# miguelmartin75/txt2vid

Measured on AMD Instinct MI355X. Metric: TGANv2 GAN train throughput (G+D steps x global batch), 16x64x64 videos/sec, higher is better.
Workload: dtype f32; 1 GPU; BASELINE configs[1]: unconditional TGANv2 16x64x64x1, per-GPU batch 32, fp32, RSGAN + GP 0.5, Adam 2e-4 (0.5,0.999), 1 D + 1 G step, subsample_input pyramid 8/16/32/64; global_batch=32, per_gpu_batch=32, parallelism=dp1

## Files before the change

### include/t2v_hip.h

```cpp
#ifndef T2V_HIP_H
#define T2V_HIP_H

#include <stddef.h>
#include <stdint.h>

#ifdef __cplusplus
extern "C" {
#endif

#define T2V_OK 0
#define T2V_EINVAL (-1)
#define T2V_ELAUNCH (-2)

#define T2V_MAX_TAPS 27

typedef struct {
    int32_t N, Cin, D, H, W, Cout;
    int32_t ntaps;
    int8_t dz[T2V_MAX_TAPS], dy[T2V_MAX_TAPS], dx[T2V_MAX_TAPS];
    int8_t pad_[3];
} t2v_conv_geom;

#define T2V_MAX_GROUPS 8
typedef struct {
// ... 28 lines not shown
    int32_t block_begin;
    int32_t bx, by;
    int8_t taps[T2V_MAX_TAPS];
    int8_t pad_[5];
} t2v_pack_job;
int t2v_pack_job_bytes(void);
int t2v_pack_job_groups(int T, int ntaps, int mode);
int t2v_pack_multi(const void* table , int njobs, int total_blocks, void* stream);

int t2v_conv_fwd(const float* x, const float* wp, const float* bias, float* y, float* ws, const t2v_conv_geom* g,
                 int flags, void* stream);
int64_t t2v_conv_fwd_ws_floats(const t2v_conv_geom* g);

int64_t t2v_conv_wgrad_slab_floats(const t2v_conv_geom* g, int T);
int t2v_conv_wgrad(const float* x, const float* gy, float* dw, float* slab, const t2v_conv_geom* g,
                   const int32_t* taps, int T, int flags, void* stream);

int64_t t2v_conv_fwd_grouped_ws_floats(const t2v_conv_group* groups, int ngroups, int Cin, int Cout);
int t2v_conv_fwd_grouped(const t2v_conv_group* groups, int ngroups, int Cin, int Cout, const float* wp,
                         const float* bias, float* ws, int flags, void* stream);
int64_t t2v_conv_wgrad_grouped_slab_floats(const t2v_conv_group* groups, int ngroups, int Cin, int Cout, int kD,
                                           int kH, int kW);
int t2v_conv_wgrad_grouped(const t2v_conv_group* groups, int ngroups, int Cin, int Cout, int kD, int kH, int kW,
                           float* dw, float* slab, int flags, void* stream);
#define T2V_WGRAD_MAX_SRC 6
typedef struct {
    const float* slab;
    const float* bias_slab;
    int32_t ntaps, S;
    int8_t map[T2V_MAX_TAPS];
    int8_t pad_[5];
    int64_t tap_stride;
    int64_t split_stride;
} t2v_wgrad_src;
typedef struct {
    float* dw;
    float* dbias;
    int64_t CoCi;
    int32_t T, Cout, nsrc;
    int32_t accum, accum_bias;
    int32_t kind;
    int32_t block_begin, nblocks;
    int32_t tap_major;
    int32_t pad_;
    t2v_wgrad_src src[T2V_WGRAD_MAX_SRC];
} t2v_wgrad_dest;
int t2v_conv_wgrad_grouped_partial(const t2v_conv_group* groups, int ngroups, int Cin, int Cout, int kD, int kH, int kW,
                                   float* slab, int want_bias, int flags, t2v_wgrad_src* out_src, void* stream);
int t2v_wgrad_dest_bytes(void);
int t2v_wgrad_reduce_multi(const void* table , int ndest, int total_blocks, void* stream);

int t2v_conv_fwd_plan(const t2v_conv_group* groups, int ngroups, int Cin, int Cout, int flags, int32_t* out);
int t2v_conv_wgrad_plan(const t2v_conv_group* groups, int ngroups, int Cin, int Cout, int kD, int kH, int kW, int32_t* out);
int64_t t2v_conv_wgrad_grouped_bias_slab_floats(const t2v_conv_group* groups, int ngroups, int Cin, int Cout, int kD,
                                                int kH, int kW);
int t2v_conv_wgrad_grouped_bias(const t2v_conv_group* groups, int ngroups, int Cin, int Cout, int kD, int kH, int kW,
                                float* dw, float* dbias, float* slab, int flags, void* stream);

int t2v_pack_weight_bf16(const float* w, void* wpb, int Cout, int Cin, int T, const int32_t* taps, int ntaps, int mode, void* stream);
int t2v_conv_fwd_grouped_bf16_ok(const t2v_conv_group* groups, int ngroups, int Cin, int Cout);
int t2v_conv_fwd_bf16_plan(const t2v_conv_group* groups, int ngroups, int Cin, int Cout, int flags, int32_t* out);
int t2v_conv_fwd_grouped_bf16(const t2v_conv_group* groups, int ngroups, int Cin, int Cout, const void* wpb, const float* bias,
                              float* ws, int flags, void* stream);

int64_t t2v_channel_sum_ws_floats(int N, int C, int64_t S);
int t2v_channel_sum(const float* x, float* out, float* ws, int N, int C, int64_t S, int accum, void* stream);
int64_t t2v_channel_sum_grouped_ws_floats(const t2v_conv_group* groups, int ngroups, int C);
int t2v_channel_sum_grouped(const t2v_conv_group* groups, int ngroups, int C, float* out, float* ws, int accum, void* stream);

int t2v_relu(const float* x, float* y, int64_t n, void* stream);
int t2v_relu_mask(const float* g, const float* x, float* gx, int64_t n, void* stream);
int t2v_add(const float* a, const float* b, float* y, int64_t n, void* stream);
int t2v_axpby(float alpha, const float* a, float beta, const float* b, float* y, int64_t n, void* stream);
int t2v_fill(float* y, float v, int64_t n, void* stream);
int t2v_tanh(const float* x, float* y, int64_t n, void* stream);
int t2v_tanh_bwd(const float* g, const float* y, float* gx, int64_t n, void* stream);

int t2v_avgpool3d(const float* x, const float* x2, float* y, int NC, int D, int H, int W, int Do, int Ho, int Wo,
                  const int32_t k[3], const int32_t s[3], const int32_t p[3], void* stream);
int t2v_avgpool3d_bwd(const float* gy, float* gx, int NC, int D, int H, int W, int Do, int Ho, int Wo,
                      const int32_t k[3], const int32_t s[3], const int32_t p[3], void* stream);
typedef struct t2v_pool_job {
    const float* x; const float* x2; float* y;
    const float* add;
    int32_t NC, D, H, W, Do, Ho, Wo;
    int32_t k[3], s[3], p[3];
} t2v_pool_job;
int t2v_avgpool3d_multi(const t2v_pool_job* jobs, int njobs, void* stream);
int t2v_avgpool3d_bwd_multi(const t2v_pool_job* jobs, int njobs, void* stream);

int t2v_rowsum(const float* x, float* y, int64_t rows, int64_t S, void* stream);
int t2v_rowbcast(const float* g, float* gx, int64_t rows, int64_t S, void* stream);

int t2v_upsample2x(const float* x, float* y, int64_t planes, int H, int W, void* stream);
int t2v_upsample2x_bwd(const float* gy, float* gx, int64_t planes, int H, int W, void* stream);
int t2v_upsample2x_add(const float* x, const float* h, float* y, int64_t planes, int H, int W, void* stream);

int64_t t2v_bn_ws_floats(int N, int C, int64_t S);
int t2v_bn_plan(int N, int C, int64_t S, int32_t* out );
int t2v_bn_stats(const float* x, float* stats, float* running_mean, float* running_var, float* ws, int N, int C,
                 int64_t S, float momentum, float eps, void* stream);
int t2v_bn_apply(const float* x, const float* stats, const float* gamma, const float* beta, float* y,
                 int N, int C, int64_t S, int relu, void* stream);
int t2v_bn_bwd(const float* gy, const float* x, const float* y, const float* stats, const float* gamma,
               float* gx, float* ggamma, float* gbeta, float* ws , int N, int C, int64_t S,
               int relu, void* stream);
// ... 278 lines not shown
```

### txt2vid_amd/_lib.py

```python
import ctypes as C
import os

_HERE = os.path.dirname(os.path.abspath(__file__))
LIB_PATH = os.environ.get('T2V_LIB') or os.path.join(_HERE, 'csrc', 'libt2v_hip.so')

MAX_TAPS = 27


class ConvGeom(C.Structure):
    _fields_ = [('N', C.c_int32), ('Cin', C.c_int32), ('D', C.c_int32), ('H', C.c_int32), ('W', C.c_int32),
                ('Cout', C.c_int32), ('ntaps', C.c_int32),
                ('dz', C.c_int8 * MAX_TAPS), ('dy', C.c_int8 * MAX_TAPS), ('dx', C.c_int8 * MAX_TAPS),
                ('pad_', C.c_int8 * 3)]


class ConvGroup(C.Structure):
    _fields_ = [('x', C.c_void_p), ('y', C.c_void_p), ('mask', C.c_void_p), ('N', C.c_int32), ('D', C.c_int32), ('H', C.c_int32), ('W', C.c_int32),
                ('ntaps', C.c_int32), ('dstride', C.c_int32), ('ydstride', C.c_int32), ('yoff', C.c_int32), ('Dy', C.c_int32),
                ('dz', C.c_int8 * MAX_TAPS), ('dy', C.c_int8 * MAX_TAPS), ('dx', C.c_int8 * MAX_TAPS), ('widx', C.c_int8 * MAX_TAPS)]


class AdamJob(C.Structure):
    _fields_ = [('p', C.c_void_p), ('g', C.c_void_p), ('m', C.c_void_p), ('v', C.c_void_p), ('n', C.c_int64)]

# ... 50 lines not shown

class AugMember(C.Structure):
    _fields_ = [('x', C.c_void_p), ('y', C.c_void_p), ('u', C.c_void_p), ('N', C.c_int32), ('C', C.c_int32), ('T', C.c_int32),
                ('S', C.c_int32), ('row_stride', C.c_int32), ('rows', C.c_int32), ('policy', C.c_int32), ('reserved', C.c_int32)]


class AdaLevel(C.Structure):
    _fields_ = [('real', C.c_void_p), ('fake', C.c_void_p), ('count', C.c_int32), ('reserved', C.c_int32)]


class LecamGrad(C.Structure):
    _fields_ = [('real', C.c_void_p), ('fake', C.c_void_p), ('d_real', C.c_void_p), ('d_fake', C.c_void_p), ('count', C.c_int32),
                ('reserved', C.c_int32)]


class ProjMember(C.Structure):
    _fields_ = [('g', C.c_void_p), ('f', C.c_void_p), ('s', C.c_void_p), ('base', C.c_void_p), ('out', C.c_void_p), ('b', C.c_int32),
                ('reserved', C.c_int32)]


class MbstdMember(C.Structure):
    _fields_ = [('f', C.c_void_p), ('g', C.c_void_p * 2), ('base', C.c_void_p * 2), ('gam', C.c_void_p), ('y', C.c_void_p * 2),
                ('stat', C.c_void_p), ('out', C.c_void_p), ('b', C.c_int32), ('seg', C.c_int32)]


MAX_GROUPS = 8
_P = C.c_void_p
_I = C.c_int
_L = C.c_int64
_F = C.c_float
_I3 = C.POINTER(C.c_int32)
_G = C.POINTER(ConvGeom)

SIGNATURES = {
    't2v_pack_weight': [_P, _P, _I, _I, _I, _I3, _I, _I, _P],
    't2v_pack_job_bytes': [],
    't2v_pack_multi': [_P, _I, _I, _P],
    't2v_pack_job_groups': [_I, _I, _I],
    't2v_pack_weight_into': [_P, _P, _I, _I, _I, _I3, _I, _I, _I, _I, _I, _I, _P],
    't2v_conv_fwd': [_P, _P, _P, _P, _P, _G, _I, _P],
    't2v_conv_fwd_ws_floats': [_G],
    't2v_conv_wgrad_slab_floats': [_G, _I],
    't2v_conv_fwd_grouped_ws_floats': [_P, _I, _I, _I],
    't2v_conv_fwd_grouped': [_P, _I, _I, _I, _P, _P, _P, _I, _P],
    't2v_conv_wgrad_grouped_slab_floats': [_P, _I, _I, _I, _I, _I, _I],
    't2v_conv_fwd_plan': [_P, _I, _I, _I, _I, _I3],
    't2v_nonlocal_ok': [_I, _I],
    't2v_nonlocal_fwd': [_P, _P, _P, _P, _P, _I, _I, _I, _I, _I, _P],
    't2v_nonlocal_bwd': [_P, _P, _P, _P, _P, _P, _P, _P, _P, _P, _I, _I, _I, _I, _I, _P],
    't2v_conv_wgrad_grouped_partial': [_P, _I, _I, _I, _I, _I, _I, _P, _I, _I, _P, _P],
    't2v_wgrad_dest_bytes': [],
    't2v_wgrad_reduce_multi': [_P, _I, _I, _P],
    't2v_conv_wgrad_plan': [_P, _I, _I, _I, _I, _I, _I, _I3],
    't2v_pack_weight_bf16': [_P, _P, _I, _I, _I, _P, _I, _I, _P],
    't2v_conv_fwd_grouped_bf16_ok': [_P, _I, _I, _I],
    't2v_conv_fwd_bf16_plan': [_P, _I, _I, _I, _I, _I3],
    't2v_conv_fwd_grouped_bf16': [_P, _I, _I, _I, _P, _P, _P, _I, _P],
    't2v_conv_wgrad_grouped': [_P, _I, _I, _I, _I, _I, _I, _P, _P, _I, _P],
    't2v_conv_wgrad_grouped_bias_slab_floats': [_P, _I, _I, _I, _I, _I, _I],
    't2v_conv_wgrad_grouped_bias': [_P, _I, _I, _I, _I, _I, _I, _P, _P, _P, _I, _P],
    't2v_conv_wgrad': [_P, _P, _P, _P, _G, _I3, _I, _I, _P],
    't2v_channel_sum_ws_floats': [_I, _I, _L],
    't2v_channel_sum': [_P, _P, _P, _I, _I, _L, _I, _P],
    't2v_channel_sum_grouped_ws_floats': [_P, _I, _I],
    't2v_channel_sum_grouped': [_P, _I, _I, _P, _P, _I, _P],
    't2v_relu': [_P, _P, _L, _P],
    't2v_relu_mask': [_P, _P, _P, _L, _P],
    't2v_add': [_P, _P, _P, _L, _P],
    't2v_axpby': [_F, _P, _F, _P, _P, _L, _P],
    't2v_fill': [_P, _F, _L, _P],
    't2v_tanh': [_P, _P, _L, _P],
    't2v_tanh_bwd': [_P, _P, _P, _L, _P],
    't2v_avgpool3d': [_P, _P, _P, _I, _I, _I, _I, _I, _I, _I, _I3, _I3, _I3, _P],
    't2v_avgpool3d_bwd': [_P, _P, _I, _I, _I, _I, _I, _I, _I, _I3, _I3, _I3, _P],
    't2v_avgpool3d_multi': [_P, _I, _P],
    't2v_avgpool3d_bwd_multi': [_P, _I, _P],
    't2v_rowsum': [_P, _P, _L, _L, _P],
    't2v_rowbcast': [_P, _P, _L, _L, _P],
    't2v_upsample2x': [_P, _P, _L, _I, _I, _P],
    't2v_upsample2x_bwd': [_P, _P, _L, _I, _I, _P],
    't2v_upsample2x_add': [_P, _P, _P, _L, _I, _I, _P],
    't2v_rsgan_mean_multi': [_P, _I, _P, _P],
    't2v_rsgan_mean_multi_bwd': [_P, _I, _P, _P],
    't2v_bn_ws_floats': [_I, _I, _L],
    't2v_bn_plan': [_I, _I, _L, _I3],
    't2v_bn_stats': [_P, _P, _P, _P, _P, _I, _I, _L, _F, _F, _P],
    't2v_bn_apply': [_P, _P, _P, _P, _P, _I, _I, _L, _I, _P],
    't2v_bn_bwd': [_P, _P, _P, _P, _P, _P, _P, _P, _P, _I, _I, _L, _I, _P],
    't2v_bn_train_fwd': [_P, _P, _P, _P, _P, _P, _P, _P, _I, _I, _L, _F, _F, _I, _P, _P],
    't2v_bn_train_bwd': [_P, _P, _P, _P, _P, _P, _P, _P, _P, _I, _I, _L, _I, _P],
    't2v_bn_train_fwd_up': [_P, _P, _P, _P, _P, _P, _P, _P, _I, _I, _I, _I, _F, _F, _I, _P, _P],
    't2v_bn_train_bwd_up': [_P, _P, _P, _P, _P, _P, _P, _P, _P, _I, _I, _I, _I, _I, _P],
    't2v_bn_train_bwd_add': [_P, _P, _P, _P, _P, _P, _P, _P, _P, _P, _I, _I, _I, _I, _I, _I, _P],
    't2v_bn_eval': [_P, _P, _P, _P, _P, _P, _I, _I, _L, _F, _I, _P],
    't2v_cbn_ws_floats': [_I, _I, _L],
    't2v_cbn_train_fwd': [_P] * 9 + [_I] * 9 + [_F, _F, _I, _P, _P],
    't2v_cbn_train_fwd_up': [_P] * 9 + [_I] * 9 + [_F, _F, _I, _P, _P],
    't2v_cbn_train_bwd': [_P] * 11 + [_I] * 9 + [_I, _P],
    't2v_cbn_train_bwd_up': [_P] * 11 + [_I] * 9 + [_I, _P],
    't2v_cbn_train_bwd_add': [_P] * 12 + [_I] * 9 + [_I, _I, _P],
    't2v_cbn_eval': [_P] * 7 + [_I] * 9 + [_F, _I, _P],
    't2v_lstm_gates': [_P, _P, _P, _P, _P, _I, _L, _P],
    't2v_lstm_gates_bwd': [_P, _P, _P, _P, _P, _P, _P, _I, _L, _P],
    't2v_skinny_gemm_splits': [_I, _I, _I],
    't2v_skinny_gemm_slab': [_P, _P, _P, _I, _I, _I, _P],
    't2v_lstm_gates_slab': [_P, _I, _P, _P, _P, _P, _P, _I, _I, _P],
# ... 125 lines not shown
```

### txt2vid_amd/csrc/conv.hip

```cpp
#include <hip/hip_runtime.h>
#include <stdint.h>
#include "../../include/t2v_hip.h"

typedef float f32x16 __attribute__((ext_vector_type(16)));

#ifdef T2V_STAMPS
__device__ unsigned long long* g_stamps = nullptr;
__device__ unsigned int g_stamps_cap = 0;
extern "C" int t2v_stamps_set(void* buf, unsigned int cap_records) {
    if (hipMemcpyToSymbol(HIP_SYMBOL(g_stamps), &buf, sizeof(buf)) != hipSuccess) return -1;
    if (hipMemcpyToSymbol(HIP_SYMBOL(g_stamps_cap), &cap_records, sizeof(cap_records)) != hipSuccess) return -1;
    return 0;
}
__device__ __forceinline__ unsigned long long stamp_now() {
    unsigned long long t;
    __builtin_amdgcn_sched_barrier(0);
    asm volatile("s_memtime %0\n\ts_waitcnt lgkmcnt(0)" : "=s"(t) :: "memory");
    __builtin_amdgcn_sched_barrier(0);
    return t;
}
#define STAMP(v) const unsigned long long v = stamp_now()
#define STAMP_ACC(acc, a, b) acc += (b) - (a)
#else
#define STAMP(v)
// ... 2369 lines not shown
        }
        if (mv) {
            py[(size_t)co * DHW] = a0;
            py[(size_t)(co + 1) * DHW] = a1;
            py[(size_t)(co + 2) * DHW] = a2;
            py[(size_t)(co + 3) * DHW] = a3;
        }
    }
}
static bool stem_ok(const t2v_conv_group* groups, int ngroups, int Cin, int Cout, int flags) {
    if ((Cin != 1 && Cin != 3) || Cout < 8 || Cout > 256 || (Cout % 4) != 0) return false;
    if (flags & (T2V_CONV_ACCUM | T2V_CONV_MASK_OUT)) return false;
    long M = 0;
    int taps = 0;
    for (int i = 0; i < ngroups; ++i) {
        if (groups[i].dstride == 2 || groups[i].ydstride == 2) return false;
        M += (long)groups[i].N * groups[i].D * groups[i].H * groups[i].W;
        if (groups[i].ntaps > taps) taps = groups[i].ntaps;
    }
    return M >= 65536 && taps > 18;
}

static bool thin_two_pass(const t2v_conv_group* groups, int ngroups, int Cin, int Cout, int nslots) {
    if (Cout != 1 || nslots < 9 || Cin < 16 || nslots * Cin > THIN_MAX_W) return false;
    long M = 0;
    for (int i = 0; i < ngroups; ++i) M += (long)groups[i].N * groups[i].D * groups[i].H * groups[i].W;
    return M >= 16384;
}

static bool thin_ok(const t2v_conv_group* groups, int ngroups, int Cin, int Cout, int& nslots) {
    if (Cout > 4) return false;
    nslots = 0;
    for (int i = 0; i < ngroups; ++i)
        for (int t = 0; t < groups[i].ntaps; ++t)
            if (groups[i].widx[t] + 1 > nslots) nslots = groups[i].widx[t] + 1;
    return (long)nslots * Cin * Cout <= THIN_MAX_W;
}

struct Tunables {
    long tile128_min;
    long tile256_min;
    long nosplit_chunks;
    long force_splits;
    long split_target;
    bool strip;
    long strip3_db;
    bool strip3_db256;
    bool occ_pad;
    long wgrad_target;
    long wgrad_scap;
    bool wgrad_quantise;
    long wgrad_min_cps;
    bool wgrad_thin;
    bool pool_fwd_db;
    bool pool_dgrad_db;
    long pool_dgrad_split_below;
    long pool_wgrad_min_cps;
};
static long env_long(const char* name, long dflt) { const char* e = getenv(name); return e ? atol(e) : dflt; }
static const Tunables& tun() {
    static const Tunables t = {env_long("T2V_TILE128_MIN", 768), env_long("T2V_TILE256_MIN", 512), env_long("T2V_NOSPLIT_CHUNKS", 8),
                               env_long("T2V_FORCE_S", 0), env_long("T2V_SPLIT_TARGET", 768), getenv("T2V_NO_STRIP") == nullptr,
                               env_long("T2V_STRIP3_DB", 16), env_long("T2V_STRIP3_DB256", 1) != 0, getenv("T2V_NO_OCC_PAD") == nullptr,
                               env_long("T2V_WGRAD_TARGET", 0), env_long("T2V_WGRAD_SCAP", 256), getenv("T2V_WGRAD_NOQ") == nullptr,
                               env_long("T2V_WGRAD_MINCPS", 4), getenv("T2V_NO_WGRAD_THIN") == nullptr,
                               env_long("T2V_POOL_FWD_DB", 1) != 0, env_long("T2V_POOL_DGRAD_DB", 0) != 0,
                               env_long("T2V_POOL_DGRAD_SPLIT_BELOW", 576), env_long("T2V_POOL_WGRAD_MINCPS", 4)};
    return t;
}

static inline int out_frames(const t2v_conv_group& g) {
    if (g.ydstride == 2) return (g.Dy + 1 - g.yoff) / 2;
    return g.dstride == 2 ? (g.D + 1) / 2 : g.D;
}
static inline long samples(const t2v_conv_group& g) { return g.N; }
static inline long voxels(const t2v_conv_group& g) { return (long)g.N * g.D * g.H * g.W; }
static inline long gemm_rows(const t2v_conv_group& g) { return (long)g.N * out_frames(g) * g.H * g.W; }

static long retile(GroupTable& tab, const t2v_conv_group* groups, int ngroups, int rows_per_tile, long (*rows_of)(const t2v_conv_group&)) {
    long mt = 0;
    for (int i = 0; i < ngroups; ++i) {
        tab.tile_start[i] = (int32_t)mt;
        mt += (rows_of(groups[i]) + rows_per_tile - 1) / rows_per_tile;
    }
    for (int i = ngroups; i <= T2V_MAX_GROUPS; ++i) tab.tile_start[i] = (int32_t)mt;
    return mt;
}

struct FwdStats { double flops = 0; long rows = 0; int taps = 0; };
static FwdStats fwd_stats(const t2v_conv_group* groups, int ngroups, int Cin, int Cout, long (*rows_of)(const t2v_conv_group&) = gemm_rows) {
    FwdStats st;
    for (int i = 0; i < ngroups; ++i) {
        st.flops += 2.0 * (double)rows_of(groups[i]) * Cout * Cin * groups[i].ntaps;
        st.rows += rows_of(groups[i]);
        if (groups[i].ntaps > st.taps) st.taps = groups[i].ntaps;
    }
    return st;
}

static void launch_splitk_reduce(const GroupTable& tab, const float* ws, const float* bias, int S, int Cin, int Cout, int flags,
                                 const FwdStats& st, hipStream_t s) {
    long blocks = (tab.out_start[tab.n] + 255) / 256;
    if (blocks > 2048) blocks = 2048;
    ProfScope prof_r(4, 0.0, s, st.rows, Cin, Cout, st.taps, tab.n, S);
    T2V_LAUNCH_PROF(splitk_reduce_kernel, dim3((unsigned)blocks), dim3(256), 0, s, tab, ws, bias, S, Cout, flags);
}

static bool group_ok(const t2v_conv_group& g, bool need_ptrs) {
    if (need_ptrs && (!g.x || !g.y)) return false;
    if (g.dstride < 0 || g.dstride > 2 || g.ydstride < 0 || g.ydstride > 2) return false;
    if (g.ydstride == 2 && (g.dstride == 2 || g.yoff < 0 || g.yoff > 1 || g.Dy < 1 || (g.Dy + 1 - g.yoff) / 2 < 1 || g.D < (g.Dy + 1) / 2)) return false;
    if (g.N < 1 || g.D < 1 || g.H < 1 || g.W < 1 || g.ntaps < 1 || g.ntaps > T2V_MAX_TAPS) return false;
    for (int t = 0; t < g.ntaps; ++t) {
        if (g.dz[t] < -1 || g.dz[t] > 1 || g.dy[t] < -1 || g.dy[t] > 1 || g.dx[t] < -1 || g.dx[t] > 1) return false;
        if (g.widx[t] < 0 || g.widx[t] >= T2V_MAX_TAPS) return false;
    }
    return true;
}
// ... 1274 lines not shown
            for (int ks = 0; ks < WG_BK / 16; ++ks) {
                const int kc = ks * 16 + 8 * hi;
                const bf16x8 a = *reinterpret_cast<const bf16x8*>(Ah + (wco * 32 + l31) * B16_KP + kc);
                const bf16x8 b0 = *reinterpret_cast<const bf16x8*>(Bh + (0 * 64 + wci * 32 + l31) * B16_KP + kc);
                const bf16x8 b1 = *reinterpret_cast<const bf16x8*>(Bh + (1 * 64 + wci * 32 + l31) * B16_KP + kc);
                const bf16x8 b2 = *reinterpret_cast<const bf16x8*>(Bh + (2 * 64 + wci * 32 + l31) * B16_KP + kc);
                acc0 = __builtin_amdgcn_mfma_f32_32x32x16_bf16(a, b0, acc0, 0, 0, 0);
                acc1 = __builtin_amdgcn_mfma_f32_32x32x16_bf16(a, b1, acc1, 0, 0, 0);
                acc2 = __builtin_amdgcn_mfma_f32_32x32x16_bf16(a, b2, acc2, 0, 0, 0);
            }
        } else {
        const float* qa = &As[(wco * 32 + l31) * W3_AP + hi];
        const float* qb = &Bs[(wci * 32 + l31) * W3_XP + 1 + hi];
#pragma unroll
        for (int k2 = 0; k2 < WG_BK / 2; ++k2) {
            const float a = qa[k2 * 2];
            const float b0 = qb[0 * 64 * W3_XP + k2 * 2];
            const float b1 = qb[1 * 64 * W3_XP + k2 * 2];
            const float b2 = qb[2 * 64 * W3_XP + k2 * 2];
            acc0 = __builtin_amdgcn_mfma_f32_32x32x2f32(a, b0, acc0, 0, 0, 0);
            acc1 = __builtin_amdgcn_mfma_f32_32x32x2f32(a, b1, acc1, 0, 0, 0);
            acc2 = __builtin_amdgcn_mfma_f32_32x32x2f32(a, b2, acc2, 0, 0, 0);
        }
        }
        __syncthreads();
    }
    if (do_bias) {
#pragma unroll
        for (int p = 0; p < 8; ++p) {
            float v = bsum[p];
#pragma unroll
            for (int o = 16; o > 0; o >>= 1) v += __shfl_xor(v, o, 64);
            const int co = co0 + rl + p * 8;
            if (ml == 0 && co < Cout) bias_slab[(size_t)split * Cout + co] = v;
        }
    }
    const int ci = ci0 + wci * 32 + l31;
    if (ci < Cin) {
        const size_t CoCi = (size_t)Cout * Cin;
        float* ps = slab + ((size_t)split * (live.n * 3) + (size_t)rslot * 3) * CoCi + ci;
#pragma unroll
        for (int r = 0; r < 16; ++r) {
            const int co = co0 + wco * 32 + (r & 3) + 8 * (r >> 2) + 4 * hi;
            if (co < Cout) {
                ps[(size_t)co * Cin] = acc0[r];
                ps[CoCi + (size_t)co * Cin] = acc1[r];
                ps[2 * CoCi + (size_t)co * Cin] = acc2[r];
            }
        }
    }
}


__global__ __launch_bounds__(256, 4) void conv_pool_wgrad_kernel(const WGroupTable tab, float* __restrict__ slab, const int Cin,
                                                              const int Cout, const int chunks_per_split, const LiveRows live,
                                                              float* __restrict__ bias_slab) {
    constexpr int PA = WG_BK + 1;
    __shared__ __attribute__((aligned(16))) float As[64 * PA];
    __shared__ __attribute__((aligned(16))) float Bs[3 * 64 * PA];
    const int tid = threadIdx.x, lane = tid & 63, wave = tid >> 6;
    const int l31 = lane & 31, hi = lane >> 5;
    const int wco = wave & 1, wci = wave >> 1;
    const int nco_t = (Cout + 63) / 64;
    const int co0 = (blockIdx.x % nco_t) * 64, ci0 = (blockIdx.x / nco_t) * 64;
    const int lin = xcd_remap((int)(blockIdx.y + blockIdx.z * gridDim.y), (int)(gridDim.y * gridDim.z));
    const int rslot = lin % (int)gridDim.y;
    const int split = lin / (int)gridDim.y;
    const int krow = live.r[rslot];
    const int dz = krow / 3 - 1, dy = krow % 3 - 1;
    const int ml = tid & 31, rl = tid >> 5;
    const bool full = co0 + 64 <= Cout && ci0 + 64 <= Cin;

    f32x16 acc0, acc1, acc2;
#pragma unroll
    for (int r = 0; r < 16; ++r) { acc0[r] = 0.f; acc1[r] = 0.f; acc2[r] = 0.f; }

    const int nchunks = tab.chunk_start[tab.n];
    const int q0 = split * chunks_per_split;
    int q1 = q0 + chunks_per_split;
    if (q1 > nchunks) q1 = nchunks;

    float ra[8], rb1[8];
    float2 rb2[8];
    bool pend_mv = false, pend_vc = false;
    const bool do_bias = bias_slab != nullptr && ci0 == 0 && rslot == 0;
    float bsum[8];
#pragma unroll
    for (int p = 0; p < 8; ++p) bsum[p] = 0.f;

    int g_i = -1, g_begin = 0, g_end = 0;
    int g_tm = 0, gHn = 1, gWn = 1, gHWn = 1, gVn = 1, gM = 0, gHp = 1, gWp = 2, gVp = 2;
    int g_lw = 0, g_lhw = 0, g_lv = 0;
    bool g_pow2 = false;
    __amdgpu_buffer_rsrc_t g_x = __builtin_amdgcn_make_buffer_rsrc((void*)tab.g[0].x, 0, 0, 0x00020000);
    __amdgpu_buffer_rsrc_t g_y = g_x;
    auto enter_group = [&](int q) {
        int gi = 0;
#pragma unroll
        for (int k = 1; k < T2V_MAX_GROUPS; ++k)
            if (k < tab.n && q >= tab.chunk_start[k]) gi = k;
        const t2v_conv_group& gd = tab.g[gi];
        g_i = gi;
        g_begin = tab.chunk_start[gi];
        g_end = tab.chunk_start[gi + 1];
        g_tm = gd.dstride;
        const int Dn = g_tm ? gd.D / 2 : 1;
// ... 392 lines not shown
    }
    for (int i = ngroups; i <= T2V_MAX_GROUPS; ++i) tab.chunk_start[i] = (int32_t)nch;
    d.nchunks = nch;
    d.nlive = __builtin_popcount(d.live);
    d.strided = strided;
    d.liverows = 0;
    for (int r = 0; r < kD * kH; ++r)
        if ((d.live >> (r * kW)) & 7u) d.liverows |= 1u << r;
    d.nrows = __builtin_popcount(d.liverows);
    const long co_tiles = (Cout + 63) / 64, tiles = co_tiles * ((Cin + 63) / 64);
    const bool rows3 = (kW == 3) && anyw && Cin >= 64 && maxMC < (1L << 30);
    if (strided && !rows3) return false;
    if (all1 && !strided && Cin >= 64 && (Cin % 4) == 0 && (Cout % 4) == 0) {
        d.kernel = WgradKernel::Gemm;
        const long t128 = (long)((Cout + 127) / 128) * ((Cin + 127) / 128);
        d.grid = dim3((unsigned)t128);
        long S = t128 >= 192 ? 1 : (256 + t128 - 1) / t128;
        const long maxS = (nch + 3) / 4;
        if (S > maxS) S = maxS;
        if (S < 1) S = 1;
        if (S > tun().wgrad_scap) S = tun().wgrad_scap;
        wgrad_set_splits(d, S, 1, Cin, Cout);
    } else if (rows3) {
        d.kernel = WgradKernel::Rows3;
        d.nlive = d.nrows * 3;
        d.grid = dim3((unsigned)tiles, (unsigned)d.nrows);
    } else if (Cin < 64 && (long)d.nlive * Cin <= 31 && tun().wgrad_thin) {
        d.kernel = WgradKernel::Thin;
        d.grid = dim3((unsigned)co_tiles);
        long S = (768 + co_tiles - 1) / co_tiles;
        const long maxS = (nch + 7) / 8;
        if (S > maxS) S = maxS;
        if (S < 1) S = 1;
        if (S > 1024) S = 1024;
        wgrad_set_splits(d, S, 4, Cin, Cout);
    } else if (Cin < 64) {
        d.kernel = WgradKernel::Cols;
        d.grid = dim3((unsigned)(co_tiles * (((long)d.nlive * Cin + 63) / 64)));
    } else {
        d.kernel = WgradKernel::Taps;
        d.grid = dim3((unsigned)tiles, (unsigned)d.nlive);
    }
    if (d.kernel != WgradKernel::Gemm && d.kernel != WgradKernel::Thin)
        wgrad_set_splits(d, wgrad_ksplit((long)d.grid.x * d.grid.y, nch, tun().wgrad_min_cps > 0 ? tun().wgrad_min_cps : 8), 1, Cin, Cout);
    d.bf16 = (flags & T2V_CONV_BF16) && (d.kernel == WgradKernel::Rows3 || d.kernel == WgradKernel::Taps);
    return true;
}

static void wgrad_plan_out(const WgradLaunch& d, int32_t* out, int n) {
    const int32_t v[8] = {(int32_t)d.kernel, d.S, d.cps, d.nlive, d.reduce_small ? 1 : 0, (int32_t)((long)d.grid.x * d.grid.y * d.grid.z),
                          d.bf16 ? 1 : 0, d.strided ? 1 : 0};
    for (int i = 0; i < n; ++i) out[i] = v[i];
}
extern "C" int t2v_conv_wgrad_plan(const t2v_conv_group* groups, int ngroups, int Cin, int Cout, int kD, int kH, int kW,
                                   int32_t* out) {
    WGroupTable tab;
    WgradLaunch d;
    if (!out || !decide_wgrad(groups, ngroups, Cin, Cout, kD, kH, kW, 0, false, tab, d)) return T2V_EINVAL;
    wgrad_plan_out(d, out, 6);
    return T2V_OK;
}
extern "C" int64_t t2v_conv_wgrad_grouped_slab_floats(const t2v_conv_group* groups, int ngroups, int Cin, int Cout, int kD,
                                                      int kH, int kW) {
    WGroupTable tab;
    WgradLaunch d;
    if (!decide_wgrad(groups, ngroups, Cin, Cout, kD, kH, kW, 0, false, tab, d)) return T2V_EINVAL;
    return d.slab_floats;
}
extern "C" int64_t t2v_conv_wgrad_grouped_bias_slab_floats(const t2v_conv_group* groups, int ngroups, int Cin, int Cout, int kD,
                                                           int kH, int kW) {
    WGroupTable tab;
    WgradLaunch d;
    if (!decide_wgrad(groups, ngroups, Cin, Cout, kD, kH, kW, 0, false, tab, d)) return T2V_EINVAL;
    return d.slab_floats + d.bias_floats;
}

static int wgrad_finish(const WgradLaunch& d, int T, const TapMap& map, float* slab, const float* bias_part, float* dw, float* dbias,
                        int Cin, int Cout, int flags, hipStream_t s, t2v_wgrad_src* out_src) {
    const long CoCi = (long)Cout * Cin;
    if (out_src) {
        out_src->slab = slab;
        out_src->bias_slab = bias_part;
        out_src->ntaps = d.nlive;
        out_src->S = d.S;
        out_src->tap_stride = CoCi;
        out_src->split_stride = (int64_t)d.nlive * CoCi;
        for (int t = 0; t < T2V_MAX_TAPS; ++t) out_src->map[t] = (int8_t)(t < T ? map.j[t] : -1);
        return T2V_OK;
    }
    const int accum = (flags & T2V_CONV_ACCUM) ? 1 : 0, accum_bias = (flags & T2V_CONV_ACCUM_BIAS) ? 1 : 0;
    ProfScope prof2(2, 0.0, s, CoCi, Cin, Cout, T, d.nlive, d.S);
    if (d.reduce_small)
        T2V_LAUNCH_PROF(wgrad_reduce_small_kernel, dim3((unsigned)((CoCi + 63) / 64), (unsigned)T), dim3(256), 0, s, slab, dw, CoCi, T,
                   d.nlive, d.S, map, accum, bias_part, dbias, Cout, accum_bias);
    else
        T2V_LAUNCH_PROF(wgrad_reduce_kernel, dim3((unsigned)((CoCi + 63) / 64)), dim3(256), 0, s, slab, dw, CoCi, T, d.nlive, d.S, map,
                   accum, bias_part, dbias, Cout, accum_bias);
    return launch_status();
}

static int wgrad_impl(const t2v_conv_group* groups, int ngroups, int Cin, int Cout, int kD, int kH, int kW, float* dw,
                      float* dbias, bool want_bias, float* slab, int flags, void* stream, t2v_wgrad_src* out_src) {
    WGroupTable tab;
    WgradLaunch d;
    if ((!dw && !out_src) || !slab || !decide_wgrad(groups, ngroups, Cin, Cout, kD, kH, kW, flags, true, tab, d)) return T2V_EINVAL;
    hipStream_t s = (hipStream_t)stream;
    float* bias_part = want_bias ? slab + d.slab_floats : (float*)nullptr;
#ifdef T2V_ABLATION
    if (const char* e = getenv("T2V_DEBUG_FLAGS")) flags |= atoi(e);
#endif
    const int T = kD * kH * kW;
    TapMap map;
    LiveTaps live;
    live.n = 0;
    for (int t = 0; t < T2V_MAX_TAPS; ++t) {
        live.t[t] = 0;
        map.j[t] = -1;
    }
    LiveRows lrows;
    lrows.n = 0;
    for (int r = 0; r < 9; ++r) lrows.r[r] = 0;
    if (d.kernel == WgradKernel::Rows3) {
        for (int r = 0; r < kD * kH; ++r)
            if ((d.liverows >> r) & 1u) {
                for (int c = 0; c < 3; ++c) map.j[r * 3 + c] = lrows.n * 3 + c;
                lrows.r[lrows.n++] = (int8_t)r;
            }
    } else {
        for (int t = 0; t < T; ++t)
            if ((d.live >> t) & 1u) { map.j[t] = live.n; live.t[live.n++] = (int8_t)t; }
    }
    double flops = 0;
    for (int i = 0; i < ngroups; ++i) {
        int live_g = 0;
        for (int a = 0; a < kD; ++a) for (int b = 0; b < kH; ++b) for (int c = 0; c < kW; ++c) {
            const int dz = a - kD / 2, dy = b - kH / 2, dx = c - kW / 2;
            if (!((groups[i].D == 1 && dz) || (groups[i].H == 1 && dy) || (groups[i].W == 1 && dx))) ++live_g;
        }
        flops += 2.0 * (double)gemm_rows(groups[i]) * Cout * Cin * live_g;
    }
    {
        ProfScope prof(1, flops, s, d.nchunks * WG_BK, Cin, Cout, d.nlive, ngroups, d.S);
        int32_t plan_[8];
        wgrad_plan_out(d, plan_, 8);
        ProfScope::set_plan(plan_, 8);
        switch (d.kernel) {
        case WgradKernel::Gemm:
            T2V_LAUNCH_PROF(conv_wgrad_gemm_kernel, d.grid, d.block, 0, s, tab, slab, Cin, Cout, flags, d.cps, bias_part);
            break;
        case WgradKernel::Rows3:
            if (d.bf16) T2V_LAUNCH_PROF(conv_wgrad3_kernel<true>, d.grid, d.block, 0, s, tab, slab, Cin, Cout, kD, kH, flags, d.cps, lrows, bias_part);
            else T2V_LAUNCH_PROF(conv_wgrad3_kernel<false>, d.grid, d.block, 0, s, tab, slab, Cin, Cout, kD, kH, flags, d.cps, lrows, bias_part);
            break;
        case WgradKernel::Thin:
            T2V_LAUNCH_PROF(conv_wgrad_thin_kernel, d.grid, d.block, 0, s, tab, slab, Cin, Cout, T, kH, kW, flags, d.cps, live, bias_part);
            break;
        case WgradKernel::Cols:
            T2V_LAUNCH_PROF(conv_wgrad_cols_kernel, d.grid, d.block, 0, s, tab, slab, Cin, Cout, T, kH, kW, flags, d.cps, live, bias_part);
            break;
        default:
            if (d.bf16) T2V_LAUNCH_PROF(conv_wgrad_bf16_kernel, d.grid, d.block, 0, s, tab, slab, Cin, Cout, T, kH, kW, flags, d.cps, live, bias_part);
            else T2V_LAUNCH_PROF(conv_wgrad_kernel, d.grid, d.block, 0, s, tab, slab, Cin, Cout, T, kH, kW, flags, d.cps, live, bias_part);
        }
    }
    int st = launch_status();
    if (st) return st;
    return wgrad_finish(d, T, map, slab, bias_part, dw, dbias, Cin, Cout, flags, s, out_src);
}
extern "C" int t2v_conv_wgrad_grouped(const t2v_conv_group* groups, int ngroups, int Cin, int Cout, int kD, int kH, int kW,
                                      float* dw, float* slab, int flags, void* stream) {
    return wgrad_impl(groups, ngroups, Cin, Cout, kD, kH, kW, dw, nullptr, false, slab, flags, stream, nullptr);
}
extern "C" int t2v_conv_wgrad_grouped_bias(const t2v_conv_group* groups, int ngroups, int Cin, int Cout, int kD, int kH, int kW,
                                           float* dw, float* dbias, float* slab, int flags, void* stream) {
    if (!dbias) return T2V_EINVAL;
    return wgrad_impl(groups, ngroups, Cin, Cout, kD, kH, kW, dw, dbias, true, slab, flags, stream, nullptr);
}

extern "C" int t2v_conv_wgrad_grouped_partial(const t2v_conv_group* groups, int ngroups, int Cin, int Cout, int kD, int kH,
                                              int kW, float* slab, int want_bias, int flags, t2v_wgrad_src* out_src,
                                              void* stream) {
    if (!out_src) return T2V_EINVAL;
    return wgrad_impl(groups, ngroups, Cin, Cout, kD, kH, kW, nullptr, nullptr, want_bias != 0, slab, flags, stream, out_src);
}
enum class PoolKernel { Fwd = 9, Dgrad = 10 };
struct PoolLaunch {
    PoolKernel kernel;
    bool db;
    bool vecb;
    int S;
    long tiles;
    dim3 grid, block;
    int64_t ws_floats;
};
static bool pool_member_ok(const t2v_conv_group& g, bool need_ptrs) {
    if (need_ptrs && (!g.x || !g.y)) return false;
    if (g.N < 1 || g.H < 2 || g.W < 2 || (g.H & 1) || (g.W & 1)) return false;
    if (g.dstride == 0) return g.D == 1;
// ... 568 lines not shown
```

Measured before the change: 3068 videos/s.

## Add specialised few-output-channel wgrad kernel with wave reductions

Adds a new weight-gradient kernel for convolutions with at most four output channels, used in place of the Rows3/Cols/Taps tile-GEMM paths when fp32 and non-strided. Each lane walks spatial positions, accumulates products of input and output gradients in registers for a slice of input channels, then reduces across the wave with DPP and shuffles. It targets the poor utilisation of GEMM tiles when Cout is tiny, such as the final RGB/output layer. It reuses the existing grid and split plan, and it relies on the assumption that the scalar per-lane loads and the full-wave reductions cost less than the wasted tile work.

```diff
diff --git a/include/t2v_hip.h b/include/t2v_hip.h
--- a/include/t2v_hip.h
+++ b/include/t2v_hip.h
@@ -104,6 +104,7 @@
 
 int t2v_conv_fwd_plan(const t2v_conv_group* groups, int ngroups, int Cin, int Cout, int flags, int32_t* out);
 int t2v_conv_wgrad_plan(const t2v_conv_group* groups, int ngroups, int Cin, int Cout, int kD, int kH, int kW, int32_t* out);
+int t2v_conv_wgrad_fewout(const t2v_conv_group* groups, int ngroups, int Cin, int Cout, int kD, int kH, int kW, int flags);
 int64_t t2v_conv_wgrad_grouped_bias_slab_floats(const t2v_conv_group* groups, int ngroups, int Cin, int Cout, int kD,
                                                 int kH, int kW);
 int t2v_conv_wgrad_grouped_bias(const t2v_conv_group* groups, int ngroups, int Cin, int Cout, int kD, int kH, int kW,
diff --git a/txt2vid_amd/_lib.py b/txt2vid_amd/_lib.py
--- a/txt2vid_amd/_lib.py
+++ b/txt2vid_amd/_lib.py
@@ -126,6 +126,7 @@
     't2v_wgrad_dest_bytes': [],
     't2v_wgrad_reduce_multi': [_P, _I, _I, _P],
     't2v_conv_wgrad_plan': [_P, _I, _I, _I, _I, _I, _I, _I3],
+    't2v_conv_wgrad_fewout': [_P, _I, _I, _I, _I, _I, _I, _I],
     't2v_pack_weight_bf16': [_P, _P, _I, _I, _I, _P, _I, _I, _P],
     't2v_conv_fwd_grouped_bf16_ok': [_P, _I, _I, _I],
     't2v_conv_fwd_bf16_plan': [_P, _I, _I, _I, _I, _I3],
diff --git a/txt2vid_amd/csrc/conv.hip b/txt2vid_amd/csrc/conv.hip
--- a/txt2vid_amd/csrc/conv.hip
+++ b/txt2vid_amd/csrc/conv.hip
@@ -2445,6 +2445,7 @@
     bool wgrad_quantise;
     long wgrad_min_cps;
     bool wgrad_thin;
+    bool wgrad_fewout;
     bool pool_fwd_db;
     bool pool_dgrad_db;
     long pool_dgrad_split_below;
@@ -2457,6 +2458,7 @@
                                env_long("T2V_STRIP3_DB", 16), env_long("T2V_STRIP3_DB256", 1) != 0, getenv("T2V_NO_OCC_PAD") == nullptr,
                                env_long("T2V_WGRAD_TARGET", 0), env_long("T2V_WGRAD_SCAP", 256), getenv("T2V_WGRAD_NOQ") == nullptr,
                                env_long("T2V_WGRAD_MINCPS", 4), getenv("T2V_NO_WGRAD_THIN") == nullptr,
+                               getenv("T2V_NO_WGRAD_FEWOUT") == nullptr,
                                env_long("T2V_POOL_FWD_DB", 1) != 0, env_long("T2V_POOL_DGRAD_DB", 0) != 0,
                                env_long("T2V_POOL_DGRAD_SPLIT_BELOW", 576), env_long("T2V_POOL_WGRAD_MINCPS", 4)};
     return t;
@@ -3837,6 +3839,194 @@
 }
 
 
+template <int CTRL>
+__device__ __forceinline__ float fo_dpp_add(float v) {
+    return v + __builtin_bit_cast(float, __builtin_amdgcn_update_dpp(0, __builtin_bit_cast(int, v), CTRL, 0xf, 0xf, true));
+}
+__device__ __forceinline__ float fo_wave_sum(float v) {
+    v = fo_dpp_add<0xB1>(v);
+    v = fo_dpp_add<0x4E>(v);
+    v = fo_dpp_add<0x141>(v);
+    v = fo_dpp_add<0x140>(v);
+    v += __shfl_xor(v, 16, 64);
+    v += __shfl_xor(v, 32, 64);
+    return v;
+}
+
+template <int KIND, int NCO>
+__global__ __launch_bounds__(256, 4) void conv_wgrad_fewout_kernel(const WGroupTable tab, float* __restrict__ slab, const int Cin,
+                                                                const int kD, const int kH, const int kW, const int flags,
+                                                                const int chunks_per_split, const LiveTaps live,
+                                                                float* __restrict__ bias_slab) {
+    constexpr int NDX = KIND == 2 ? 3 : 1;
+    constexpr int CH = NCO == 1 ? (KIND == 2 ? 8 : 16) : NCO == 2 ? 8 : 4;
+    constexpr int NJ = CH * NDX;
+    constexpr int NCTX = KIND == 2 ? 3 : KIND == 0 ? 1 : CH;
+    const int lane = threadIdx.x & 63;
+    const int wave = __builtin_amdgcn_readfirstlane((int)(threadIdx.x >> 6));
+    const int lin = xcd_remap((int)(blockIdx.y + blockIdx.z * gridDim.y), (int)(gridDim.y * gridDim.z));
+    const int yslot = lin % (int)gridDim.y;
+    const int split = lin / (int)gridDim.y;
+    const int nslots = live.n, ncols = nslots * Cin;
+    const int T = kD * kH * kW;
+    const bool relu_in = flags & T2V_CONV_RELU_IN;
+    const int nchunks = tab.chunk_start[tab.n];
+    const int q0 = split * chunks_per_split;
+    int q1 = q0 + chunks_per_split;
+    if (q1 > nchunks) q1 = nchunks;
+    const bool do_bias = bias_slab != nullptr && blockIdx.x == 0 && wave == 0 &&
+                         (KIND == 1 || (KIND == 2 ? yslot == 0 : (int)live.t[yslot] == T / 2));
+    float bsum[NCO];
+#pragma unroll
+    for (int co = 0; co < NCO; ++co) bsum[co] = 0.f;
+
+    for (int pass = 0; pass < 16 / CH; ++pass) {
+        const int cb = (int)blockIdx.x * 64 + wave * 16 + pass * CH;
+        int c_ci[CH], x_dz[NCTX], x_dy[NCTX], x_dx[NCTX];
+        int x_slot[NCTX] = {0};
+#pragma unroll
+        for (int c = 0; c < CH; ++c) {
+            if (KIND == 1) {
+                const bool ok = cb + c < ncols;
+                x_slot[c % NCTX] = ok ? (cb + c) / Cin : 0;
+                c_ci[c] = ok ? cb + c - x_slot[c % NCTX] * Cin : 0;
+            } else {
+                c_ci[c] = cb + c < Cin ? cb + c : Cin - 1;
+            }
+        }
+#pragma unroll
+        for (int k = 0; k < NCTX; ++k) {
+            const int t = live.t[KIND == 1 ? x_slot[k] : KIND == 2 ? yslot * 3 + k : yslot];
+            x_dz[k] = t / (kH * kW) - kD / 2;
+            x_dy[k] = (t / kW) % kH - kH / 2;
+            x_dx[k] = t % kW - kW / 2;
+        }
+        float acc[NJ][NCO];
+#pragma unroll
+        for (int j = 0; j < NJ; ++j)
+#pragma unroll
+            for (int co = 0; co < NCO; ++co) acc[j][co] = 0.f;
+
+        int q = q0;
+        while (q < q1) {
+            int gi = 0;
+#pragma unroll
+            for (int k = 1; k < T2V_MAX_GROUPS; ++k)
+                if (k < tab.n && q >= tab.chunk_start[k]) gi = k;
+            const t2v_conv_group& gd = tab.g[gi];
+            const int g_begin = tab.chunk_start[gi];
+            int qe = tab.chunk_start[gi + 1];
+            if (qe > q1) qe = q1;
+            const int D = gd.D, H = gd.H, W = gd.W, HW = H * W, DHW = D * HW, gM = gd.N * DHW;
+            const bool pow2 = ((D & (D - 1)) | (H & (H - 1)) | (W & (W - 1))) == 0;
+            const int lw = __builtin_ctz(W), lhw = lw + __builtin_ctz(H);
+            const bool small = gM < (1 << 24);
+            const float rDHW = 1.0f / (float)DHW, rHW = 1.0f / (float)HW, rW = 1.0f / (float)W;
+            int x_shift[NCTX];
+#pragma unroll
+            for (int k = 0; k < NCTX; ++k) x_shift[k] = x_dz[k] * HW + x_dy[k] * W + x_dx[k];
+            const __amdgpu_buffer_rsrc_t g_x =
+                __builtin_amdgcn_make_buffer_rsrc((void*)gd.x, 0, (int)((uint32_t)gM * (uint32_t)Cin * 4u), 0x00020000);
+            const __amdgpu_buffer_rsrc_t g_y =
+                __builtin_amdgcn_make_buffer_rsrc((void*)gd.y, 0, (int)((uint32_t)gM * (uint32_t)NCO * 4u), 0x00020000);
+            int v1 = (qe - g_begin) * WG_BK;
+            if (v1 > gM) v1 = gM;
+            for (int vb = (q - g_begin) * WG_BK; vb < v1; vb += 64) {
+                const int m = vb + lane;
+                const bool mv = m < v1;
+                int sp, d, h, w_;
+                if (pow2) {
+                    sp = m & (DHW - 1);
+                    d = sp >> lhw;
+                    h = (sp >> lw) & (H - 1);
+                    w_ = sp & (W - 1);
+                } else {
+                    const int n = small ? fast_div(m, DHW, rDHW) : m / DHW;
+                    sp = m - n * DHW;
+                    d = small ? fast_div(sp, HW, rHW) : sp / HW;
+                    const int r = sp - d * HW;
+                    h = small ? fast_div(r, W, rW) : r / W;
+                    w_ = r - h * W;
+                }
+                const uint32_t gb = mv ? (uint32_t)(m - sp) * (uint32_t)NCO + (uint32_t)sp : 0u;
+                const uint32_t xb = (uint32_t)(m - sp) * (uint32_t)Cin + (uint32_t)sp;
+                float gy[NCO], xv[NJ];
+                bool val[NCTX];
+                uint32_t voff[NCTX];
+#pragma unroll
+                for (int co = 0; co < NCO; ++co)
+                    gy[co] = __builtin_bit_cast(float, __builtin_amdgcn_raw_buffer_load_b32(g_y, (gb + (uint32_t)(co * DHW)) * 4u, 0, 0));
+#pragma unroll
+                for (int k = 0; k < NCTX; ++k) {
+                    val[k] = mv && (unsigned)(d + x_dz[k]) < (unsigned)D && (unsigned)(h + x_dy[k]) < (unsigned)H &&
+                             (unsigned)(w_ + x_dx[k]) < (unsigned)W;
+                    voff[k] = val[k] ? (xb + (uint32_t)x_shift[k]) * 4u : 0u;
+                }
+#pragma unroll
+                for (int j = 0; j < NJ; ++j)
+                    xv[j] = __builtin_bit_cast(float, __builtin_amdgcn_raw_buffer_load_b32(
+                        g_x, voff[KIND == 1 ? j : j % NDX], (int)((uint32_t)c_ci[j / NDX] * (uint32_t)DHW * 4u), 0));
+                if (relu_in) {
+#pragma unroll
+                    for (int j = 0; j < NJ; ++j) xv[j] = fmaxf(xv[j], 0.f);
+                }
+                float gm[NCTX][NCO];
+#pragma unroll
+                for (int k = 0; k < NCTX; ++k)
+#pragma unroll
+                    for (int co = 0; co < NCO; ++co) gm[k][co] = val[k] ? gy[co] : 0.f;
+#pragma unroll
+                for (int j = 0; j < NJ; ++j)
+#pragma unroll
+                    for (int co = 0; co < NCO; ++co)
+                        acc[j][co] = __builtin_fmaf(gm[KIND == 1 ? j : j % NDX][co], xv[j], acc[j][co]);
+                if (do_bias && pass == 0) {
+#pragma unroll
+                    for (int co = 0; co < NCO; ++co) bsum[co] += mv ? gy[co] : 0.f;
+                }
+            }
+            q = qe;
+        }
+
+        float outv[NCO];
+#pragma unroll
+        for (int co = 0; co < NCO; ++co) outv[co] = 0.f;
+#pragma unroll
+        for (int j = 0; j < NJ; ++j)
+#pragma unroll
+            for (int co = 0; co < NCO; ++co) {
+                const float s = fo_wave_sum(acc[j][co]);
+                outv[co] = lane == j ? s : outv[co];
+            }
+        int slot, ci;
+        bool ok = lane < NJ;
+        if (KIND == 1) {
+            const int col = cb + lane;
+            ok = ok && col < ncols;
+            slot = ok ? col / Cin : 0;
+            ci = col - slot * Cin;
+        } else {
+            const int c = lane / NDX;
+            ci = cb + c;
+            ok = ok && ci < Cin;
+            slot = KIND == 2 ? yslot * 3 + (lane - c * NDX) : yslot;
+        }
+        if (ok) {
+            float* ps = slab + (((size_t)split * nslots + slot) * NCO) * Cin + ci;
+#pragma unroll
+            for (int co = 0; co < NCO; ++co) ps[(size_t)co * Cin] = outv[co];
+        }
+    }
+    if (do_bias) {
+#pragma unroll
+        for (int co = 0; co < NCO; ++co) {
+            const float s = fo_wave_sum(bsum[co]);
+            if (lane == 0) bias_slab[(size_t)split * NCO + co] = s;
+        }
+    }
+}
+
+
 __global__ __launch_bounds__(256, 4) void conv_pool_wgrad_kernel(const WGroupTable tab, float* __restrict__ slab, const int Cin,
                                                               const int Cout, const int chunks_per_split, const LiveRows live,
                                                               float* __restrict__ bias_slab) {
@@ -4335,6 +4525,16 @@
                           d.bf16 ? 1 : 0, d.strided ? 1 : 0};
     for (int i = 0; i < n; ++i) out[i] = v[i];
 }
+static bool wgrad_fewout(const WgradLaunch& d, int Cout, int flags) {
+    return tun().wgrad_fewout && Cout <= 4 && !(flags & T2V_CONV_BF16) && !d.strided &&
+           (d.kernel == WgradKernel::Rows3 || d.kernel == WgradKernel::Cols || d.kernel == WgradKernel::Taps);
+}
+extern "C" int t2v_conv_wgrad_fewout(const t2v_conv_group* groups, int ngroups, int Cin, int Cout, int kD, int kH, int kW, int flags) {
+    WGroupTable tab;
+    WgradLaunch d;
+    if (!decide_wgrad(groups, ngroups, Cin, Cout, kD, kH, kW, flags, false, tab, d)) return T2V_EINVAL;
+    return wgrad_fewout(d, Cout, flags) ? 1 : 0;
+}
 extern "C" int t2v_conv_wgrad_plan(const t2v_conv_group* groups, int ngroups, int Cin, int Cout, int kD, int kH, int kW,
                                    int32_t* out) {
     WGroupTable tab;
@@ -4426,7 +4626,24 @@
         ProfScope prof(1, flops, s, d.nchunks * WG_BK, Cin, Cout, d.nlive, ngroups, d.S);
         int32_t plan_[8];
         wgrad_plan_out(d, plan_, 8);
+        const bool fewout = wgrad_fewout(d, Cout, flags);
+        if (fewout) plan_[6] = 2;
         ProfScope::set_plan(plan_, 8);
+        if (fewout) {
+            LiveTaps fl = live;
+            if (d.kernel == WgradKernel::Rows3) {
+                fl.n = lrows.n * 3;
+                for (int r = 0; r < lrows.n; ++r)
+                    for (int c = 0; c < 3; ++c) fl.t[r * 3 + c] = (int8_t)(lrows.r[r] * 3 + c);
+            }
+#define T2V_FEWOUT_CASE(K, N) case N: T2V_LAUNCH_PROF((conv_wgrad_fewout_kernel<K, N>), d.grid, d.block, 0, s, tab, slab, Cin, kD, kH, kW, flags, d.cps, fl, bias_part); break;
+#define T2V_FEWOUT_KIND(K) switch (Cout) { T2V_FEWOUT_CASE(K, 1) T2V_FEWOUT_CASE(K, 2) T2V_FEWOUT_CASE(K, 3) T2V_FEWOUT_CASE(K, 4) }
+            if (d.kernel == WgradKernel::Rows3) T2V_FEWOUT_KIND(2)
+            else if (d.kernel == WgradKernel::Cols) T2V_FEWOUT_KIND(1)
+            else T2V_FEWOUT_KIND(0)
+#undef T2V_FEWOUT_KIND
+#undef T2V_FEWOUT_CASE
+        } else
         switch (d.kernel) {
         case WgradKernel::Gemm:
             T2V_LAUNCH_PROF(conv_wgrad_gemm_kernel, d.grid, d.block, 0, s, tab, slab, Cin, Cout, flags, d.cps, bias_part);
```

New measurement: 3087 videos/s (median of 6 runs). No clear change (+0.6%).
